# alibaba/TorchEasyRec

Hardware: NVIDIA H100
Metric: samples/sec (DLRM-Criteo synth, train step fwd+bwd+optimizer) (higher is better)
Workload: dtype f32

## Files before the change

### torcheasyrec_b200/csrc/build.py

```python

import os
import subprocess
import sys

HERE = os.path.dirname(os.path.abspath(__file__))
SOURCES = ["tzk_core.cu", "tzk_gather.cu", "tzk_bwd.cu", "tzk_dist.cu", "tzk_dense.cu", "tzk_tower.cu", "tzk_din.cu", "tzk_peer.cu", "tzk_interact_wide.cu",
           "tzk_interact_bf16.cu"]
HEADERS = ["tzk_common.cuh", "tzk_tower_bwd2.cuh", "tzk_interact_tc.cuh", "tzk_tower_tail.cuh", "tzk_interact_bf16.cuh",
"tzk_sm90_ptx.h", "tzk_tma.h", "tzk_wgrad3x.cuh", os.path.join("..", "..", "include", "tzk.h")]
LIB = os.path.join(HERE, "libtzk.so")
NVCC = os.environ.get("NVCC", "/usr/local/cuda/bin/nvcc")
FLAGS = [
    "-gencode", "arch=compute_90a,code=sm_90a",
    "-O3", "-lineinfo", "-std=c++17",
    "-Xcompiler", "-fPIC",
    "--expt-relaxed-constexpr",
]


def _mtime(p):
    return os.path.getmtime(p) if os.path.exists(p) else 0.0


def build(verbose: bool = False, force: bool = False) -> str:
    hdr_time = max(_mtime(os.path.join(HERE, h)) for h in HEADERS)
    objs = []
    procs = []
    for src in SOURCES:
        s = os.path.join(HERE, src)
        o = os.path.join(HERE, src.replace(".cu", ".o"))
        objs.append(o)
        if force or _mtime(o) < max(_mtime(s), hdr_time):
            cmd = [NVCC, *FLAGS, "-c", s, "-o", o]
            if verbose:
                cmd.insert(1, "-Xptxas")
                cmd.insert(2, "-v")
                print(" ".join(cmd), flush=True)
            procs.append((src, subprocess.Popen(cmd, stdout=subprocess.PIPE, stderr=subprocess.STDOUT, text=True)))
    failed = False
    for src, p in procs:
        out, _ = p.communicate()
        if p.returncode != 0:
            failed = True
            sys.stderr.write(f"nvcc failed for {src}:\n{out}\n")
        elif verbose and out:
            print(out)
    if failed:
        raise RuntimeError("libtzk build failed")
    if force or procs or _mtime(LIB) < max(_mtime(o) for o in objs):
        cmd = [NVCC, "-shared", "-Wno-deprecated-gpu-targets", "-o", LIB + ".tmp", *objs]
        subprocess.run(cmd, check=True)
        os.replace(LIB + ".tmp", LIB)
    build_gemm(force)
    build_gemm3x(force)
    return LIB


def build_gemm3x(force: bool = False) -> str:
    src = os.path.join(HERE, "tzk_gemm3x.cu")
    lib = os.path.join(HERE, "libtzk_gemm3x.so")
    deps = [src] + [os.path.join(HERE, h) for h in ("tzk_sm90_ptx.h", "tzk_tma.h", "tzk_wgrad3x.cuh")]
    if force or _mtime(lib) < max(_mtime(d) for d in deps):
        subprocess.run([NVCC, *FLAGS, "-shared", src, "-o", lib + ".tmp"], check=True)
        os.replace(lib + ".tmp", lib)
    return lib


def build_gemm(force: bool = False) -> str:
    src = os.path.join(HERE, "tzk_gemm.cpp")
    lib = os.path.join(HERE, "libtzk_gemm.so")
    if force or _mtime(lib) < _mtime(src):
        subprocess.run(["g++", "-O2", "-std=c++17", "-fPIC", "-shared", "-I/usr/local/cuda/include", src, "-o", lib,
                        "-ldl"], check=True)
    return lib


if __name__ == "__main__":
    print(build(verbose="-v" in sys.argv, force="-f" in sys.argv))
```

### torcheasyrec_b200/csrc/tzk_interact_wide.cu

```cuda
#include <stdint.h>
#include <stdio.h>
#include <stdlib.h>

#ifdef TZK_CPU_SHIM
#include "cuda_cpu_shim.h"
#include "sm90_cpu_emu.h"
typedef void* tzk_stream_t;
#define TZK_REQUIRE(cond, ...) do { if (!(cond)) return 1; } while (0)
#define TZK_CHECK_LAUNCH(name) do {} while (0)
#else
#include <cuda.h>
#include "tzk_common.cuh"
#define TZK_DYN_SMEM(type, name) extern __shared__ __align__(1024) type name[]
#define TZK_UNPAREN(...) __VA_ARGS__
#define TZK_LAUNCH(kernel, grid, block, smem, stream, ...) TZK_UNPAREN kernel<<<grid, block, smem, stream>>>(__VA_ARGS__)
#endif

namespace {
#ifndef TZK_CPU_SHIM
#include "tzk_sm90_ptx.h"
#endif
#include "tzk_tma.h"
namespace tzk_itc {
__device__ __forceinline__ uint32_t cvt_tf32(float x) { return tf32_bits(x); }
__device__ __forceinline__ void mma_tf32(float (&c)[4], const uint32_t (&a)[4], const uint32_t (&b)[2]) { ::mma_tf32(c, a, b); }
}
#include "tzk_interact_tc.cuh"

__device__ __forceinline__ float4 load_l2(const float* p) {
#ifdef TZK_CPU_SHIM
  return *reinterpret_cast<const float4*>(p);
#else
  return __ldcg(reinterpret_cast<const float4*>(p));
#endif
}

constexpr int FB_M = 64;
constexpr int FB_THREADS = 512;
constexpr int FB_WARPS = FB_THREADS / 32;
constexpr int FB_CHUNKS = (tzk_itc::kRow + 31) / 32;
constexpr int FB_PAIR_CHUNKS = tzk_itc::kInter / 32;
constexpr int FB_BOX = 32 * 128;
constexpr int FB_STAGE = 4 * FB_BOX;
constexpr int FB_STAGES = 3;
constexpr int FB_LDP = 360;
constexpr int FB_P_OFF = FB_STAGES * FB_STAGE;
constexpr int FB_S_OFF = FB_P_OFF + FB_M * FB_LDP * 4;
constexpr int FB_IJ_OFF = FB_S_OFF + FB_WARPS * 32 * tzk_itc::kSS * 4;
constexpr int FB_BAR_OFF = FB_IJ_OFF + tzk_itc::kInter * 2;
constexpr int FB_SMEM = FB_BAR_OFF + FB_STAGES * 8;

struct FbParams {
  const float* dz; int64_t ld_dz;
  const float* dense; int64_t ld_dense;
  const float* sparse; int64_t ld_sparse;
  float* d_dense; int64_t ld_ddense;
  float* d_sparse; int64_t ld_dsparse;
  int64_t M;
};

__global__ void __launch_bounds__(FB_THREADS, 1)
interact_wide_bwd_kernel(const __grid_constant__ CUtensorMap map_whi, const __grid_constant__ CUtensorMap map_wlo,
                         FbParams p) {
  TZK_DYN_SMEM(uint8_t, smem);
  float* P = reinterpret_cast<float*>(smem + FB_P_OFF);
  uint64_t* full = reinterpret_cast<uint64_t*>(smem + FB_BAR_OFF);
  const int warp = threadIdx.x >> 5, lane = threadIdx.x & 31, g = lane >> 2, t = lane & 3;
  const int64_t m0 = (int64_t)blockIdx.x * FB_M;

  if (threadIdx.x == 0) {
    for (int s = 0; s < FB_STAGES; ++s) mbar_init(full + s, 1);
    fence_mbarrier_init();
  }
  float* S = reinterpret_cast<float*>(smem + FB_S_OFF) + warp * (32 * tzk_itc::kSS);
  unsigned short* pair_ij = reinterpret_cast<unsigned short*>(smem + FB_IJ_OFF);
  tzk_itc::init_pair_ij(pair_ij);
  for (int i = lane; i < 32 * tzk_itc::kSS; i += 32) S[i] = 0.f;
  __syncthreads();
  auto col_chunk = [](int c) { return (c + FB_PAIR_CHUNKS) % FB_CHUNKS; };
  auto load = [&](int c) {
    uint8_t* sb = smem + (c % FB_STAGES) * FB_STAGE;
    uint64_t* bar = full + c % FB_STAGES;
    const int n0 = col_chunk(c) * 32;
    mbar_expect_tx(bar, FB_STAGE);
    tma_load_2d(sb, &map_whi, bar, 0, n0);
    tma_load_2d(sb + FB_BOX, &map_whi, bar, 32, n0);
    tma_load_2d(sb + 2 * FB_BOX, &map_wlo, bar, 0, n0);
    tma_load_2d(sb + 3 * FB_BOX, &map_wlo, bar, 32, n0);
  };
  if (threadIdx.x == 0)
    for (int c = 0; c < FB_STAGES; ++c) load(c);

  const int wm = warp & 3, wn = warp >> 2;
  const int r = wm * 16 + g;
  uint32_t ah[8][4], al[8][4];
#pragma unroll
  for (int kk = 0; kk < 8; ++kk) {
    const int k0 = kk * 8 + t, k1 = k0 + 4;
    const int64_t ra = m0 + r, rb = ra + 8;
    const float a[4] = {ra < p.M ? __ldg(p.dz + ra * p.ld_dz + k0) : 0.f, rb < p.M ? __ldg(p.dz + rb * p.ld_dz + k0) : 0.f,
                        ra < p.M ? __ldg(p.dz + ra * p.ld_dz + k1) : 0.f, rb < p.M ? __ldg(p.dz + rb * p.ld_dz + k1) : 0.f};
#pragma unroll
    for (int i = 0; i < 4; ++i) {
      ah[kk][i] = tf32_bits(a[i]);
      al[kk][i] = tf32_bits(a[i] - __uint_as_float(ah[kk][i]));
    }
  }
  const int n = wn * 8 + g;
  for (int c = 0; c < FB_CHUNKS; ++c) {
    const int s = c % FB_STAGES;
    mbar_wait(full + s, (uint32_t)(c / FB_STAGES) & 1u);
    const uint32_t* whi = reinterpret_cast<const uint32_t*>(smem + s * FB_STAGE);
    const uint32_t* wlo = whi + 2 * FB_BOX / 4;
    float acc[4] = {0.f, 0.f, 0.f, 0.f};
#pragma unroll
    for (int kk = 0; kk < 8; ++kk) {
      const uint32_t* bh_box = whi + (kk >> 2) * (FB_BOX / 4);
      const uint32_t* bl_box = wlo + (kk >> 2) * (FB_BOX / 4);
      const int k0 = (kk & 3) * 8 + t, k1 = k0 + 4;
      const uint32_t bh[2] = {bh_box[swz(n, k0)], bh_box[swz(n, k1)]};
      const uint32_t bl[2] = {bl_box[swz(n, k0)], bl_box[swz(n, k1)]};
      float part[4] = {0.f, 0.f, 0.f, 0.f};
      mma_tf32(part, al[kk], bh);
      mma_tf32(part, ah[kk], bl);
      mma_tf32(part, ah[kk], bh);
#pragma unroll
      for (int q = 0; q < 4; ++q) acc[q] += part[q];
    }
    const int col = col_chunk(c) * 32 + wn * 8 + 2 * t;
    if (col < tzk_itc::kInter) {
      *reinterpret_cast<float2*>(P + r * FB_LDP + col) = make_float2(acc[0], acc[1]);
      *reinterpret_cast<float2*>(P + (r + 8) * FB_LDP + col) = make_float2(acc[2], acc[3]);
    } else if (col < tzk_itc::kRow) {
      const int e = col - tzk_itc::kInter;
#pragma unroll
      for (int h = 0; h < 2; ++h) {
        const int64_t row = m0 + r + 8 * h;
        if (row >= p.M) continue;
        float* dst = e < tzk_itc::kD ? p.d_dense + row * p.ld_ddense + e : p.d_sparse + row * p.ld_dsparse + (e - tzk_itc::kD);
        *reinterpret_cast<float2*>(dst) = make_float2(acc[2 * h], acc[2 * h + 1]);
      }
    }
    __syncthreads();
    if (threadIdx.x == 0 && c + FB_STAGES < FB_CHUNKS) load(c + FB_STAGES);
  }

  for (int i = warp; i < FB_M; i += FB_WARPS) {
    const int64_t b = m0 + i;
    if (b >= p.M) break;
    float* dd = p.d_dense + b * p.ld_ddense;
    float* ds = p.d_sparse + b * p.ld_dsparse;
    float4 pass[4];
#pragma unroll
    for (int q = 0; q < 4; ++q) {
      const int row = g + 8 * q;
      pass[q] = row == 0 ? load_l2(dd + 4 * t)
              : row < tzk_itc::kN ? load_l2(ds + (row - 1) * tzk_itc::kD + 4 * t)
              : make_float4(0.f, 0.f, 0.f, 0.f);
    }
    tzk_itc::bwd_sample(P + i * FB_LDP, p.dense + b * p.ld_dense, p.sparse + b * p.ld_sparse, pass, pair_ij, S, dd, ds,
                        lane);
  }
}

constexpr int FF_M = 128;
constexpr int FF_THREADS = 256;
constexpr int FF_WARPS = FF_THREADS / 32;
constexpr int FF_X_BYTES = FF_M * 128;
constexpr int FF_W_BYTES = 64 * 128;
constexpr int FF_STAGE = FF_X_BYTES + 2 * FF_W_BYTES;
constexpr int FF_STAGES = 3;
constexpr int FF_E_OFF = FF_STAGES * FF_STAGE;
constexpr int FF_BAR_OFF = FF_E_OFF + FF_X_BYTES;
constexpr int FF_SMEM = FF_BAR_OFF + FF_STAGES * 8;
static_assert(FF_WARPS * tzk_itc::kInter * 4 <= FF_X_BYTES, "staging rows overflow their region");
constexpr int FF_SPARSE0 = tzk_itc::kInter + tzk_itc::kD;

struct FfParams {
  const float* dense; int64_t ld_dense;
  const float* sparse; int64_t ld_sparse;
  float* pairs; int64_t ld_pairs;
  const float* bias;
  float* y; int64_t ld_y;
  int64_t M;
};

__device__ __forceinline__ void fence_proxy_async() {
#ifndef TZK_CPU_SHIM
  asm volatile("fence.proxy.async;" ::: "memory");
#endif
}

__global__ void __launch_bounds__(FF_THREADS, 2)
interact_wide_fwd_kernel(const __grid_constant__ CUtensorMap map_pairs, const __grid_constant__ CUtensorMap map_dense,
                         const __grid_constant__ CUtensorMap map_sparse, const __grid_constant__ CUtensorMap map_whi, const __grid_constant__ CUtensorMap map_wlo,
                         FfParams p) {
  TZK_DYN_SMEM(uint8_t, smem);
  uint64_t* full = reinterpret_cast<uint64_t*>(smem + FF_BAR_OFF);
  const int warp = threadIdx.x >> 5, lane = threadIdx.x & 31, g = lane >> 2, t = lane & 3;
  const int64_t m0 = (int64_t)blockIdx.x * FF_M;
  const int64_t m_end = p.M - m0 < FF_M ? p.M : m0 + FF_M;

  if (threadIdx.x == 0) {
    for (int s = 0; s < FF_STAGES; ++s) mbar_init(full + s, 1);
    fence_mbarrier_init();
  }
  {
    float* O = reinterpret_cast<float*>(smem + FF_E_OFF) + warp * tzk_itc::kInter;
    if (lane == 0) O[tzk_itc::kP] = 0.f;
    int rowbase[4];
    tzk_itc::pair_rowbase(g, rowbase);
    int64_t b = m0 + warp;
    float4 x[4];
    if (b < m_end) {
#pragma unroll
      for (int j = 0; j < 4; ++j) x[j] = tzk_itc::load_x4(p.dense + b * p.ld_dense, p.sparse + b * p.ld_sparse, g + 8 * j, 4 * t);
    }
    for (; b < m_end; b += FF_WARPS) {
      float4 xn[4];
      const int64_t bn = b + FF_WARPS;
      if (bn < m_end) {
#pragma unroll
        for (int j = 0; j < 4; ++j)
          xn[j] = tzk_itc::load_x4(p.dense + bn * p.ld_dense, p.sparse + bn * p.ld_sparse, g + 8 * j, 4 * t);
      }
      tzk_itc::fwd_sample(x, rowbase, O, p.pairs + b * p.ld_pairs, lane);
      if (bn < m_end) {
#pragma unroll
        for (int j = 0; j < 4; ++j) x[j] = xn[j];
      }
    }
  }
  fence_proxy_async();
  __syncthreads();

  auto load = [&](int c) {
    uint8_t* sb = smem + (c % FF_STAGES) * FF_STAGE;
    uint64_t* bar = full + c % FF_STAGES;
    mbar_expect_tx(bar, c == FB_PAIR_CHUNKS ? FF_STAGE + FF_X_BYTES : FF_STAGE);
    if (c < FB_PAIR_CHUNKS) {
      tma_load_2d(sb, &map_pairs, bar, 32 * c, (int)m0);
    } else if (c == FB_PAIR_CHUNKS) {
      tma_load_2d(sb, &map_dense, bar, 0, (int)m0);
      tma_load_2d(smem + FF_E_OFF, &map_sparse, bar, 0, (int)m0);
    } else {
      tma_load_2d(sb, &map_sparse, bar, 32 * c - FF_SPARSE0, (int)m0);
    }
    tma_load_2d(sb + FF_X_BYTES, &map_whi, bar, 32 * c, 0);
    tma_load_2d(sb + FF_X_BYTES + FF_W_BYTES, &map_wlo, bar, 32 * c, 0);
  };
  if (threadIdx.x == 0)
    for (int c = 0; c < FF_STAGES; ++c) load(c);

  const int r = warp * 16 + g;
  float acc[8][4], part[8][4];
#pragma unroll
  for (int nt = 0; nt < 8; ++nt)
#pragma unroll
    for (int q = 0; q < 4; ++q) acc[nt][q] = 0.f;
  for (int c = 0; c < FB_CHUNKS; ++c) {
    const int s = c % FF_STAGES;
    mbar_wait(full + s, (uint32_t)(c / FF_STAGES) & 1u);
    const float* xs = reinterpret_cast<const float*>(smem + s * FF_STAGE);
    const uint32_t* whi = reinterpret_cast<const uint32_t*>(smem + s * FF_STAGE + FF_X_BYTES);
    const uint32_t* wlo = whi + FF_W_BYTES / 4;
#pragma unroll
    for (int ks = 0; ks < 4; ++ks) {
#pragma unroll
      for (int nt = 0; nt < 8; ++nt)
#pragma unroll
        for (int q = 0; q < 4; ++q) part[nt][q] = 0.f;
      const int k0 = ks * 8 + t, k1 = k0 + 4;
      const bool sp = ks >= 2 && c == FB_PAIR_CHUNKS;
      const float* as = sp ? reinterpret_cast<const float*>(smem + FF_E_OFF) : xs;
      const int x16 = sp ? 16 : 0;
      const float a[4] = {as[swz(r, k0) ^ x16], as[swz(r + 8, k0) ^ x16], as[swz(r, k1) ^ x16], as[swz(r + 8, k1) ^ x16]};
      uint32_t ah[4], al[4];
#pragma unroll
      for (int i = 0; i < 4; ++i) {
        ah[i] = tf32_bits(a[i]);
        al[i] = tf32_bits(a[i] - __uint_as_float(ah[i]));
      }
#pragma unroll
      for (int nt = 0; nt < 8; ++nt) {
        const int n = nt * 8 + g;
        const uint32_t bh[2] = {whi[swz(n, k0)], whi[swz(n, k1)]};
        const uint32_t bl[2] = {wlo[swz(n, k0)], wlo[swz(n, k1)]};
        mma_tf32(part[nt], al, bh);
        mma_tf32(part[nt], ah, bl);
        mma_tf32(part[nt], ah, bh);
      }
#pragma unroll
      for (int nt = 0; nt < 8; ++nt)
#pragma unroll
        for (int q = 0; q < 4; ++q) acc[nt][q] += part[nt][q];
    }
    __syncthreads();
    if (threadIdx.x == 0 && c + FF_STAGES < FB_CHUNKS) load(c + FF_STAGES);
  }
#pragma unroll
  for (int nt = 0; nt < 8; ++nt) {
    const int col = nt * 8 + 2 * t;
    const float b0 = p.bias ? __ldg(p.bias + col) : 0.f, b1 = p.bias ? __ldg(p.bias + col + 1) : 0.f;
#pragma unroll
    for (int h = 0; h < 2; ++h) {
      const int64_t row = m0 + r + 8 * h;
      if (row >= p.M) continue;
      float2 o = make_float2(acc[nt][2 * h] + b0, acc[nt][2 * h + 1] + b1);
      o.x = fmaxf(o.x, 0.f);
      o.y = fmaxf(o.y, 0.f);
      *reinterpret_cast<float2*>(p.y + row * p.ld_y + col) = o;
    }
  }
}

__global__ void split_w_kernel(const float* __restrict__ w, int64_t ld_w, int K, float* __restrict__ hi,
                               float* __restrict__ lo) {
  const int i = blockIdx.x * blockDim.x + threadIdx.x;
  if (i < K * 64) {
    const float v = w[(int64_t)(i / K) * ld_w + i % K];
    const float h = tf32_rna(v);
    hi[i] = h;
    lo[i] = tf32_rna(v - h);
  }
}

#include "tzk_wgrad3x.cuh"

__global__ void split_wt_kernel(const float* __restrict__ w, int64_t ld_w, int K, float* __restrict__ hi,
                                float* __restrict__ lo) {
  const int i = blockIdx.x * blockDim.x + threadIdx.x;
  if (i < K * 64) {
    const int k = i >> 6, o = i & 63;
    const float v = w[(int64_t)o * ld_w + k];
    const float h = tf32_rna(v);
    hi[i] = h;
    lo[i] = tf32_rna(v - h);
  }
}

}

extern "C" int tzk_interact_wide_bwd(const float* dz, int64_t ld_dz, const float* w, int64_t ld_w, const float* dense,
                                     int64_t ld_dense, const float* sparse, int64_t ld_sparse, int64_t M, float* d_dense,
                                     int64_t ld_ddense, float* d_sparse, int64_t ld_dsparse, float* wt_hi, float* wt_lo,
                                     tzk_stream_t stream) {
  TZK_REQUIRE(M > 0, "interact_wide_bwd: M must be positive");
  TZK_REQUIRE(ld_w >= tzk_itc::kRow, "interact_wide_bwd: w needs %d columns", tzk_itc::kRow);
  const int64_t lds[] = {ld_dz, ld_w, ld_dense, ld_sparse, ld_ddense, ld_dsparse};
  for (int64_t ld : lds) TZK_REQUIRE(ld % 4 == 0, "interact_wide_bwd: row strides must be multiples of 4 floats");
  const void* ptrs[] = {dz, w, dense, sparse, d_dense, d_sparse, wt_hi, wt_lo};
  for (const void* q : ptrs)
    TZK_REQUIRE(q && reinterpret_cast<uintptr_t>(q) % 16 == 0, "interact_wide_bwd: NULL or not 16-B aligned pointer");
  cudaStream_t st = reinterpret_cast<cudaStream_t>(stream);
  TZK_LAUNCH((split_wt_kernel), (tzk_itc::kRow * 64 + 255) / 256, 256, 0, st, w, ld_w, tzk_itc::kRow, wt_hi, wt_lo);
  CUtensorMap mh, ml;
  TZK_REQUIRE(!make_map(&mh, wt_hi, tzk_itc::kRow, 64, 64, 32) && !make_map(&ml, wt_lo, tzk_itc::kRow, 64, 64, 32),
              "interact_wide_bwd: tensor-map encoding failed");
  FbParams p;
  p.dz = dz; p.ld_dz = ld_dz; p.dense = dense; p.ld_dense = ld_dense; p.sparse = sparse; p.ld_sparse = ld_sparse;
  p.d_dense = d_dense; p.ld_ddense = ld_ddense; p.d_sparse = d_sparse; p.ld_dsparse = ld_dsparse; p.M = M;
#ifndef TZK_CPU_SHIM
  static bool configured = false;
  if (!configured) {
    cudaFuncSetAttribute(interact_wide_bwd_kernel, cudaFuncAttributeMaxDynamicSharedMemorySize, FB_SMEM);
    configured = true;
  }
#endif
  TZK_LAUNCH((interact_wide_bwd_kernel), (unsigned)((M + FB_M - 1) / FB_M), FB_THREADS, FB_SMEM, st, mh, ml, p);
  TZK_CHECK_LAUNCH("interact_wide_bwd_kernel");
  return 0;
}

extern "C" int tzk_interact_wide_fwd(const float* dense, int64_t ld_dense, const float* sparse, int64_t ld_sparse,
                                     const float* w, int64_t ld_w, const float* bias, int64_t M, float* y, int64_t ld_y,
                                     float* pairs, int64_t ld_pairs, float* w_hi, float* w_lo, tzk_stream_t stream) {
  TZK_REQUIRE(M > 0, "interact_wide_fwd: M must be positive");
  TZK_REQUIRE(ld_w >= tzk_itc::kRow && ld_y >= 64 && ld_pairs >= tzk_itc::kInter && ld_dense >= tzk_itc::kD &&
              ld_sparse >= tzk_itc::kRow - FF_SPARSE0, "interact_wide_fwd: row stride shorter than the row");
  const int64_t lds[] = {ld_dense, ld_sparse, ld_w, ld_y, ld_pairs};
  for (int64_t ld : lds) TZK_REQUIRE(ld % 4 == 0, "interact_wide_fwd: row strides must be multiples of 4 floats");
  const void* ptrs[] = {dense, sparse, w, y, pairs, w_hi, w_lo};
  for (const void* q : ptrs)
    TZK_REQUIRE(q && reinterpret_cast<uintptr_t>(q) % 16 == 0, "interact_wide_fwd: NULL or not 16-B aligned pointer");
  cudaStream_t st = reinterpret_cast<cudaStream_t>(stream);
  TZK_LAUNCH((split_w_kernel), (tzk_itc::kRow * 64 + 255) / 256, 256, 0, st, w, ld_w, tzk_itc::kRow, w_hi, w_lo);
  CUtensorMap mp, md, ms, mh, ml;
  TZK_REQUIRE(!make_map(&mp, pairs, M, tzk_itc::kInter, ld_pairs, FF_M) &&
              !make_map(&md, dense, M, tzk_itc::kD, ld_dense, FF_M) &&
              !make_map(&ms, sparse, M, tzk_itc::kRow - FF_SPARSE0, ld_sparse, FF_M) &&
              !make_map(&mh, w_hi, 64, tzk_itc::kRow, tzk_itc::kRow, 64) &&
              !make_map(&ml, w_lo, 64, tzk_itc::kRow, tzk_itc::kRow, 64), "interact_wide_fwd: tensor-map encoding failed");
  FfParams p;
  p.dense = dense; p.ld_dense = ld_dense; p.sparse = sparse; p.ld_sparse = ld_sparse; p.pairs = pairs;
  p.ld_pairs = ld_pairs; p.bias = bias; p.y = y; p.ld_y = ld_y; p.M = M;
#ifndef TZK_CPU_SHIM
  static bool configured = false;
  if (!configured) {
    cudaFuncSetAttribute(interact_wide_fwd_kernel, cudaFuncAttributeMaxDynamicSharedMemorySize, FF_SMEM);
    configured = true;
  }
#endif
  TZK_LAUNCH((interact_wide_fwd_kernel), (unsigned)((M + FF_M - 1) / FF_M), FF_THREADS, FF_SMEM, st, mp, md, ms, mh, ml, p);
  TZK_CHECK_LAUNCH("interact_wide_fwd_kernel");
  return 0;
}

extern "C" int tzk_interact_wide_wgrad(const float* dz, int64_t ld_dz, const float* pairs, int64_t ld_pairs,
                                       const float* dense, int64_t ld_dense, const float* sparse, int64_t ld_sparse,
                                       int64_t M, int32_t slabs, float* partial, float* dw, int64_t ld_dw,
                                       tzk_stream_t stream) {
  TZK_REQUIRE(M > 0 && slabs > 0, "interact_wide_wgrad: M and slabs must be positive");
  TZK_REQUIRE(ld_dw >= tzk_itc::kRow, "interact_wide_wgrad: dw needs %d columns", tzk_itc::kRow);
  const int64_t lds[] = {ld_dz, ld_pairs, ld_dense, ld_sparse};
  for (int64_t ld : lds) TZK_REQUIRE(ld % 4 == 0, "interact_wide_wgrad: row strides must be multiples of 4 floats");
  const void* ptrs[] = {dz, pairs, dense, sparse, partial, dw};
  for (const void* q : ptrs)
    TZK_REQUIRE(q && reinterpret_cast<uintptr_t>(q) % 16 == 0, "interact_wide_wgrad: NULL or not 16-B aligned pointer");
  CUtensorMap mx[WG_SRC], mz;
  TZK_REQUIRE(!make_map(&mx[0], pairs, M, tzk_itc::kInter, ld_pairs, WG_ROWS) &&
              !make_map(&mx[1], sparse, M, tzk_itc::kRow - FF_SPARSE0, ld_sparse, WG_ROWS) &&
              !make_map(&mx[2], dense, M, tzk_itc::kD, ld_dense, WG_ROWS) &&
              !make_map(&mz, dz, M, 64, ld_dz, WG_ROWS), "interact_wide_wgrad: tensor-map encoding failed");
  const WgSources src = {{0, FB_PAIR_CHUNKS, FB_CHUNKS - 1, FB_CHUNKS}, {0, 0, 0}, {0, FF_SPARSE0, tzk_itc::kInter},
                         {tzk_itc::kInter, tzk_itc::kRow - FF_SPARSE0, tzk_itc::kD}};
  TZK_REQUIRE(wgrad3x_launch(mx, mz, src, M, slabs, partial, dw, ld_dw, reinterpret_cast<cudaStream_t>(stream)) == 0,
              "interact_wide_wgrad: launch failed");
  return 0;
}
```

### torcheasyrec_b200/csrc/tzk_wgrad3x.cuh

```cuda
#pragma once

constexpr int WG_THREADS = 256;
constexpr int WG_ROWS = 32;
constexpr int WG_BOX = WG_ROWS * 128;
constexpr int WG_A = 4 * WG_BOX, WG_B = 2 * WG_BOX;
constexpr int WG_STAGE = WG_A + WG_B;
constexpr int WG_STAGES = 4;
constexpr int WG_SRC = 3;

struct WgSources {
  int first[WG_SRC + 1];
  int col0[WG_SRC];
  int dst[WG_SRC];
  int width[WG_SRC];
};

struct WgParams {
  float* partial;
  int64_t M;
  int64_t slab_rows;
  int k_tiles;
  WgSources src;
};

__device__ __forceinline__ int wg_source(const WgSources& s, int box) {
  return box >= s.first[2] ? 2 : box >= s.first[1] ? 1 : 0;
}
__device__ __forceinline__ int wg_pick(const int* v, int s) { return s == 0 ? v[0] : s == 1 ? v[1] : v[2]; }

__global__ void __launch_bounds__(WG_THREADS, 2)
wgrad3x_kernel(const __grid_constant__ CUtensorMap map_x0, const __grid_constant__ CUtensorMap map_x1,
               const __grid_constant__ CUtensorMap map_x2, const __grid_constant__ CUtensorMap map_dz, WgParams p) {
  TZK_DYN_SMEM(uint8_t, smem);
  uint64_t* full = reinterpret_cast<uint64_t*>(smem + WG_STAGES * WG_STAGE);
  int* boxes = reinterpret_cast<int*>(full + WG_STAGES);

  const int warp = threadIdx.x >> 5, lane = threadIdx.x & 31, g = lane >> 2, t = lane & 3;
  const int jt = blockIdx.x % p.k_tiles;
  const int64_t slab = blockIdx.x / p.k_tiles;
  const int64_t row0 = slab * p.slab_rows;
  const int64_t rows = (p.M - row0 < p.slab_rows) ? p.M - row0 : p.slab_rows;
  const int num_c = (int)((rows + WG_ROWS - 1) / WG_ROWS);

  if (threadIdx.x == 0) {
    for (int s = 0; s < WG_STAGES; ++s) mbar_init(full + s, 1);
    fence_mbarrier_init();
    for (int b = 0; b < 4; ++b) {
      const int box = jt * 4 + b, s = wg_source(p.src, box);
      boxes[b] = s;
      boxes[4 + b] = wg_pick(p.src.col0, s) + 32 * (box - wg_pick(p.src.first, s));
    }
  }
  __syncthreads();
  auto load = [&](int c) {
    uint8_t* sb = smem + (c % WG_STAGES) * WG_STAGE;
    uint64_t* bar = full + c % WG_STAGES;
    const int r = (int)(row0 + (int64_t)c * WG_ROWS);
    mbar_expect_tx(bar, WG_A + WG_B);
#pragma unroll 1
    for (int b = 0; b < 4; ++b) {
      const int s = *reinterpret_cast<volatile int*>(boxes + b), col = *reinterpret_cast<volatile int*>(boxes + 4 + b);
      tma_load_2d(sb + b * WG_BOX, s == 0 ? &map_x0 : s == 1 ? &map_x1 : &map_x2, bar, col, r);
    }
#pragma unroll
    for (int b = 0; b < 2; ++b) tma_load_2d(sb + WG_A + b * WG_BOX, &map_dz, bar, b * 32, r);
  };
  if (threadIdx.x == 0)
    for (int c = 0; c < WG_STAGES && c < num_c; ++c) load(c);

  const int n0 = (warp & 3) * 16 + g;
  const int kc0 = (warp >> 2) * 64 + g;
  float acc[8][4], part[8][4];
#pragma unroll
  for (int nt = 0; nt < 8; ++nt)
#pragma unroll
    for (int q = 0; q < 4; ++q) acc[nt][q] = 0.f;
  for (int c = 0; c < num_c; ++c) {
    const int s = c % WG_STAGES;
    mbar_wait(full + s, (uint32_t)(c / WG_STAGES) & 1u);
    const float* xs = reinterpret_cast<const float*>(smem + s * WG_STAGE);
    const float* zs = reinterpret_cast<const float*>(smem + s * WG_STAGE + WG_A);
    auto at = [](const float* base, int m, int col) { return base[(col >> 5) * (WG_BOX / 4) + swz(m, col & 31)]; };
#pragma unroll
    for (int ks = 0; ks < WG_ROWS / 8; ++ks) {
#pragma unroll
      for (int nt = 0; nt < 8; ++nt)
#pragma unroll
        for (int q = 0; q < 4; ++q) part[nt][q] = 0.f;
      const int m = ks * 8 + t;
      const float a[4] = {at(zs, m, n0), at(zs, m, n0 + 8), at(zs, m + 4, n0), at(zs, m + 4, n0 + 8)};
      uint32_t ah[4], al[4];
#pragma unroll
      for (int i = 0; i < 4; ++i) {
        ah[i] = tf32_bits(a[i]);
        al[i] = tf32_bits(a[i] - __uint_as_float(ah[i]));
      }
#pragma unroll
      for (int nt = 0; nt < 8; ++nt) {
        const float b[2] = {at(xs, m, kc0 + 8 * nt), at(xs, m + 4, kc0 + 8 * nt)};
        uint32_t bh[2], bl[2];
#pragma unroll
        for (int i = 0; i < 2; ++i) {
          bh[i] = tf32_bits(b[i]);
          bl[i] = tf32_bits(b[i] - __uint_as_float(bh[i]));
        }
        mma_tf32(part[nt], al, bh);
        mma_tf32(part[nt], ah, bl);
        mma_tf32(part[nt], ah, bh);
      }
#pragma unroll
      for (int nt = 0; nt < 8; ++nt)
#pragma unroll
        for (int q = 0; q < 4; ++q) acc[nt][q] += part[nt][q];
    }
    __syncthreads();
    if (threadIdx.x == 0 && c + WG_STAGES < num_c) load(c + WG_STAGES);
  }
  float* out = p.partial + ((int64_t)slab * p.k_tiles + jt) * 128 * 64;
#pragma unroll
  for (int nt = 0; nt < 8; ++nt) {
    const int kcol = (warp >> 2) * 64 + nt * 8 + 2 * t;
#pragma unroll
    for (int q = 0; q < 4; ++q) out[(int64_t)(kcol + (q & 1)) * 64 + n0 + 8 * (q >> 1)] = acc[nt][q];
  }
}

__global__ void wgrad_reduce_kernel(const float* __restrict__ partial, int slabs, int k_pad, WgSources src,
                                    float* __restrict__ dw, int64_t ld_dw) {
  const int i = blockIdx.x * blockDim.x + threadIdx.x;
  if (i >= k_pad * 64) return;
  const int k = i >> 6, n = i & 63;
  const int s = wg_source(src, k >> 5);
  const int c = k - 32 * wg_pick(src.first, s);
  if (c >= wg_pick(src.width, s)) return;
  float acc = 0.f;
  for (int sl = 0; sl < slabs; ++sl) acc += partial[((int64_t)sl * k_pad + k) * 64 + n];
  dw[(int64_t)n * ld_dw + wg_pick(src.dst, s) + c] = acc;
}

inline int wgrad3x_launch(const CUtensorMap (&mx)[WG_SRC], const CUtensorMap& mz, const WgSources& src, int64_t M,
                          int32_t slabs, float* partial, float* dw, int64_t ld_dw, cudaStream_t st) {
  WgParams p;
  p.partial = partial;
  p.M = M;
  p.k_tiles = (src.first[WG_SRC] + 3) / 4;
  p.slab_rows = ((M + slabs - 1) / slabs + WG_ROWS - 1) / WG_ROWS * WG_ROWS;
  p.src = src;
  const int used = (int)((M + p.slab_rows - 1) / p.slab_rows);
  const size_t smem = (size_t)WG_STAGES * WG_STAGE + WG_STAGES * 8 + 8 * 4;
#ifndef TZK_CPU_SHIM
  static bool configured = false;
  if (!configured) {
    cudaFuncSetAttribute(wgrad3x_kernel, cudaFuncAttributeMaxDynamicSharedMemorySize, (int)smem);
    configured = true;
  }
#endif
  TZK_LAUNCH((wgrad3x_kernel), used * p.k_tiles, WG_THREADS, smem, st, mx[0], mx[1], mx[2], mz, p);
  TZK_LAUNCH((wgrad_reduce_kernel), (p.k_tiles * 128 * 64 + 255) / 256, 256, 0, st, partial, used, p.k_tiles * 128, src,
             dw, ld_dw);
  return cudaGetLastError() == cudaSuccess ? 0 : 3;
}
```

Before: 45.83 million.

## Use wgmma 3xTF32 for interact-wide forward and weight-gradient GEMMs

Replaces the warp-level mma.sync 3xTF32 loops in the interact-wide forward kernel with Hopper wgmma m64n64k8 instructions that read the B operand (weight hi/lo) directly from swizzled shared memory through descriptors. Adds a dedicated weight-gradient kernel that splits dz into tf32 hi/lo transposed tiles in shared memory each chunk, then issues wgmma against them, and templatizes the wgrad launcher to accept this kernel and its extra smem. The aim is to cut shared-memory fragment loads and per-warp MMA issue overhead. In exchange it adds an extra smem staging pass and syncs per chunk, raises smem use (which can lower occupancy), and waits on each wgmma group immediately, so there is little async overlap.

```diff
diff --git a/torcheasyrec_b200/csrc/build.py b/torcheasyrec_b200/csrc/build.py
--- a/torcheasyrec_b200/csrc/build.py
+++ b/torcheasyrec_b200/csrc/build.py
@@ -7,7 +7,7 @@
 SOURCES = ["tzk_core.cu", "tzk_gather.cu", "tzk_bwd.cu", "tzk_dist.cu", "tzk_dense.cu", "tzk_tower.cu", "tzk_din.cu", "tzk_peer.cu", "tzk_interact_wide.cu",
            "tzk_interact_bf16.cu"]
 HEADERS = ["tzk_common.cuh", "tzk_tower_bwd2.cuh", "tzk_interact_tc.cuh", "tzk_tower_tail.cuh", "tzk_interact_bf16.cuh",
-"tzk_sm90_ptx.h", "tzk_tma.h", "tzk_wgrad3x.cuh", os.path.join("..", "..", "include", "tzk.h")]
+"tzk_sm90_ptx.h", "tzk_tma.h", "tzk_wgrad3x.cuh", "tzk_wgmma.cuh", os.path.join("..", "..", "include", "tzk.h")]
 LIB = os.path.join(HERE, "libtzk.so")
 NVCC = os.environ.get("NVCC", "/usr/local/cuda/bin/nvcc")
 FLAGS = [
diff --git a/torcheasyrec_b200/csrc/tzk_interact_wide.cu b/torcheasyrec_b200/csrc/tzk_interact_wide.cu
--- a/torcheasyrec_b200/csrc/tzk_interact_wide.cu
+++ b/torcheasyrec_b200/csrc/tzk_interact_wide.cu
@@ -5,6 +5,7 @@
 #ifdef TZK_CPU_SHIM
 #include "cuda_cpu_shim.h"
 #include "sm90_cpu_emu.h"
+#include "sm90_wgmma_emu.h"
 typedef void* tzk_stream_t;
 #define TZK_REQUIRE(cond, ...) do { if (!(cond)) return 1; } while (0)
 #define TZK_CHECK_LAUNCH(name) do {} while (0)
@@ -21,6 +22,7 @@
 #include "tzk_sm90_ptx.h"
 #endif
 #include "tzk_tma.h"
+#include "tzk_wgmma.cuh"
 namespace tzk_itc {
 __device__ __forceinline__ uint32_t cvt_tf32(float x) { return tf32_bits(x); }
 __device__ __forceinline__ void mma_tf32(float (&c)[4], const uint32_t (&a)[4], const uint32_t (&b)[2]) { ::mma_tf32(c, a, b); }
@@ -253,23 +255,17 @@
     for (int c = 0; c < FF_STAGES; ++c) load(c);
 
   const int r = warp * 16 + g;
-  float acc[8][4], part[8][4];
-#pragma unroll
-  for (int nt = 0; nt < 8; ++nt)
-#pragma unroll
-    for (int q = 0; q < 4; ++q) acc[nt][q] = 0.f;
+  float acc[32], part[32];
+#pragma unroll
+  for (int i = 0; i < 32; ++i) acc[i] = 0.f;
   for (int c = 0; c < FB_CHUNKS; ++c) {
     const int s = c % FF_STAGES;
     mbar_wait(full + s, (uint32_t)(c / FF_STAGES) & 1u);
     const float* xs = reinterpret_cast<const float*>(smem + s * FF_STAGE);
-    const uint32_t* whi = reinterpret_cast<const uint32_t*>(smem + s * FF_STAGE + FF_X_BYTES);
-    const uint32_t* wlo = whi + FF_W_BYTES / 4;
+    const uint8_t* whi = smem + s * FF_STAGE + FF_X_BYTES;
+    const uint8_t* wlo = whi + FF_W_BYTES;
 #pragma unroll
     for (int ks = 0; ks < 4; ++ks) {
-#pragma unroll
-      for (int nt = 0; nt < 8; ++nt)
-#pragma unroll
-        for (int q = 0; q < 4; ++q) part[nt][q] = 0.f;
       const int k0 = ks * 8 + t, k1 = k0 + 4;
       const bool sp = ks >= 2 && c == FB_PAIR_CHUNKS;
       const float* as = sp ? reinterpret_cast<const float*>(smem + FF_E_OFF) : xs;
@@ -281,19 +277,15 @@
         ah[i] = tf32_bits(a[i]);
         al[i] = tf32_bits(a[i] - __uint_as_float(ah[i]));
       }
-#pragma unroll
-      for (int nt = 0; nt < 8; ++nt) {
-        const int n = nt * 8 + g;
-        const uint32_t bh[2] = {whi[swz(n, k0)], whi[swz(n, k1)]};
-        const uint32_t bl[2] = {wlo[swz(n, k0)], wlo[swz(n, k1)]};
-        mma_tf32(part[nt], al, bh);
-        mma_tf32(part[nt], ah, bl);
-        mma_tf32(part[nt], ah, bh);
-      }
-#pragma unroll
-      for (int nt = 0; nt < 8; ++nt)
-#pragma unroll
-        for (int q = 0; q < 4; ++q) acc[nt][q] += part[nt][q];
+      wgmma_fence();
+      wgmma_3xtf32<64>(part, ah, al, wgmma_desc(whi, ks), wgmma_desc(wlo, ks));
+      wgmma_commit();
+      wgmma_wait<0>();
+#pragma unroll
+      for (int i = 0; i < 32; ++i) {
+        wgmma_reg_fence(part[i]);
+        acc[i] += part[i];
+      }
     }
     __syncthreads();
     if (threadIdx.x == 0 && c + FF_STAGES < FB_CHUNKS) load(c + FF_STAGES);
@@ -306,7 +298,7 @@
     for (int h = 0; h < 2; ++h) {
       const int64_t row = m0 + r + 8 * h;
       if (row >= p.M) continue;
-      float2 o = make_float2(acc[nt][2 * h] + b0, acc[nt][2 * h + 1] + b1);
+      float2 o = make_float2(acc[4 * nt + 2 * h] + b0, acc[4 * nt + 2 * h + 1] + b1);
       o.x = fmaxf(o.x, 0.f);
       o.y = fmaxf(o.y, 0.f);
       *reinterpret_cast<float2*>(p.y + row * p.ld_y + col) = o;
@@ -326,6 +318,112 @@
 }
 
 #include "tzk_wgrad3x.cuh"
+
+constexpr int WW_ZT = 64 * 128;
+
+__global__ void __launch_bounds__(WG_THREADS, 2)
+interact_wide_wgrad_kernel(const __grid_constant__ CUtensorMap map_x0, const __grid_constant__ CUtensorMap map_x1,
+                           const __grid_constant__ CUtensorMap map_x2, const __grid_constant__ CUtensorMap map_dz,
+                           WgParams p) {
+  TZK_DYN_SMEM(uint8_t, smem);
+  uint8_t* zt = smem + WG_STAGES * WG_STAGE;
+  uint64_t* full = reinterpret_cast<uint64_t*>(zt + 2 * WW_ZT);
+  int* boxes = reinterpret_cast<int*>(full + WG_STAGES);
+
+  const int warp = threadIdx.x >> 5, lane = threadIdx.x & 31, g = lane >> 2, t = lane & 3;
+  const int jt = blockIdx.x % p.k_tiles;
+  const int64_t slab = blockIdx.x / p.k_tiles;
+  const int64_t row0 = slab * p.slab_rows;
+  const int64_t rows = (p.M - row0 < p.slab_rows) ? p.M - row0 : p.slab_rows;
+  const int num_c = (int)((rows + WG_ROWS - 1) / WG_ROWS);
+
+  if (threadIdx.x == 0) {
+    for (int s = 0; s < WG_STAGES; ++s) mbar_init(full + s, 1);
+    fence_mbarrier_init();
+    for (int b = 0; b < 4; ++b) {
+      const int box = jt * 4 + b, s = wg_source(p.src, box);
+      boxes[b] = s;
+      boxes[4 + b] = wg_pick(p.src.col0, s) + 32 * (box - wg_pick(p.src.first, s));
+    }
+  }
+  __syncthreads();
+  auto load = [&](int c) {
+    uint8_t* sb = smem + (c % WG_STAGES) * WG_STAGE;
+    uint64_t* bar = full + c % WG_STAGES;
+    const int r = (int)(row0 + (int64_t)c * WG_ROWS);
+    mbar_expect_tx(bar, WG_A + WG_B);
+#pragma unroll 1
+    for (int b = 0; b < 4; ++b) {
+      const int s = *reinterpret_cast<volatile int*>(boxes + b), col = *reinterpret_cast<volatile int*>(boxes + 4 + b);
+      tma_load_2d(sb + b * WG_BOX, s == 0 ? &map_x0 : s == 1 ? &map_x1 : &map_x2, bar, col, r);
+    }
+#pragma unroll
+    for (int b = 0; b < 2; ++b) tma_load_2d(sb + WG_A + b * WG_BOX, &map_dz, bar, b * 32, r);
+  };
+  if (threadIdx.x == 0)
+    for (int c = 0; c < WG_STAGES && c < num_c; ++c) load(c);
+
+  const int xc = (warp >> 2) * 64 + (warp & 3) * 16 + g;
+  const int tn = threadIdx.x & 63, tq = threadIdx.x >> 6;
+  uint32_t* zhi = reinterpret_cast<uint32_t*>(zt);
+  uint32_t* zlo = zhi + WW_ZT / 4;
+  float acc[32], part[32];
+#pragma unroll
+  for (int i = 0; i < 32; ++i) acc[i] = 0.f;
+  for (int c = 0; c < num_c; ++c) {
+    const int s = c % WG_STAGES;
+    mbar_wait(full + s, (uint32_t)(c / WG_STAGES) & 1u);
+    const float* xs = reinterpret_cast<const float*>(smem + s * WG_STAGE);
+    const float* zs = reinterpret_cast<const float*>(smem + s * WG_STAGE + WG_A);
+    auto at = [](const float* base, int m, int col) { return base[(col >> 5) * (WG_BOX / 4) + swz(m, col & 31)]; };
+#pragma unroll
+    for (int h = 0; h < 2; ++h) {
+      const int m = 4 * tq + 16 * h;
+      float hi[4], lo[4];
+#pragma unroll
+      for (int j = 0; j < 4; ++j) {
+        const float v = at(zs, m + j, tn);
+        hi[j] = tf32_rna(v);
+        lo[j] = tf32_rna(v - hi[j]);
+      }
+      *reinterpret_cast<float4*>(zhi + swz(tn, m)) = make_float4(hi[0], hi[1], hi[2], hi[3]);
+      *reinterpret_cast<float4*>(zlo + swz(tn, m)) = make_float4(lo[0], lo[1], lo[2], lo[3]);
+    }
+    fence_proxy_async();
+    __syncthreads();
+#pragma unroll
+    for (int ks = 0; ks < WG_ROWS / 8; ++ks) {
+      const int m = ks * 8 + t;
+      const float a[4] = {at(xs, m, xc), at(xs, m, xc + 8), at(xs, m + 4, xc), at(xs, m + 4, xc + 8)};
+      uint32_t ah[4], al[4];
+#pragma unroll
+      for (int i = 0; i < 4; ++i) {
+        ah[i] = tf32_bits(a[i]);
+        al[i] = tf32_bits(a[i] - __uint_as_float(ah[i]));
+      }
+      wgmma_fence();
+      wgmma_tf32<64>(part, ah, wgmma_desc(zlo, ks), false);
+      wgmma_tf32<64>(part, al, wgmma_desc(zhi, ks), true);
+      wgmma_tf32<64>(part, ah, wgmma_desc(zhi, ks), true);
+      wgmma_commit();
+      wgmma_wait<0>();
+#pragma unroll
+      for (int i = 0; i < 32; ++i) {
+        wgmma_reg_fence(part[i]);
+        acc[i] += part[i];
+      }
+    }
+    __syncthreads();
+    if (threadIdx.x == 0 && c + WG_STAGES < num_c) load(c + WG_STAGES);
+  }
+  float* out = p.partial + ((int64_t)slab * p.k_tiles + jt) * 128 * 64;
+#pragma unroll
+  for (int i = 0; i < 8; ++i)
+#pragma unroll
+    for (int h = 0; h < 2; ++h)
+      *reinterpret_cast<float2*>(out + (int64_t)(xc + 8 * h) * 64 + 8 * i + 2 * t) =
+          make_float2(acc[4 * i + 2 * h], acc[4 * i + 2 * h + 1]);
+}
 
 __global__ void split_wt_kernel(const float* __restrict__ w, int64_t ld_w, int K, float* __restrict__ hi,
                                 float* __restrict__ lo) {
@@ -424,7 +522,8 @@
               !make_map(&mz, dz, M, 64, ld_dz, WG_ROWS), "interact_wide_wgrad: tensor-map encoding failed");
   const WgSources src = {{0, FB_PAIR_CHUNKS, FB_CHUNKS - 1, FB_CHUNKS}, {0, 0, 0}, {0, FF_SPARSE0, tzk_itc::kInter},
                          {tzk_itc::kInter, tzk_itc::kRow - FF_SPARSE0, tzk_itc::kD}};
-  TZK_REQUIRE(wgrad3x_launch(mx, mz, src, M, slabs, partial, dw, ld_dw, reinterpret_cast<cudaStream_t>(stream)) == 0,
+  TZK_REQUIRE(wgrad3x_launch<interact_wide_wgrad_kernel>(mx, mz, src, M, slabs, partial, dw, ld_dw,
+                                                         reinterpret_cast<cudaStream_t>(stream), 2 * WW_ZT) == 0,
               "interact_wide_wgrad: launch failed");
   return 0;
 }
diff --git a/torcheasyrec_b200/csrc/tzk_wgmma.cuh b/torcheasyrec_b200/csrc/tzk_wgmma.cuh
--- /dev/null
+++ b/torcheasyrec_b200/csrc/tzk_wgmma.cuh
@@ -0,0 +1,39 @@
+#pragma once
+
+__device__ __forceinline__ uint64_t wgmma_desc(const void* box, int ks) {
+  const uint32_t a = smem_u32(box) + 32u * (uint32_t)ks;
+  return (uint64_t)((a >> 4) & 0x3fffu) | (1ull << 16) | ((uint64_t)(1024 >> 4) << 32) | (1ull << 62);
+}
+
+#ifndef TZK_CPU_SHIM
+__device__ __forceinline__ void wgmma_fence() { asm volatile("wgmma.fence.sync.aligned;" ::: "memory"); }
+__device__ __forceinline__ void wgmma_commit() { asm volatile("wgmma.commit_group.sync.aligned;" ::: "memory"); }
+template <int N>
+__device__ __forceinline__ void wgmma_wait() { asm volatile("wgmma.wait_group.sync.aligned %0;" ::"n"(N) : "memory"); }
+__device__ __forceinline__ void wgmma_reg_fence(float& r) { asm volatile("" : "+f"(r)::"memory"); }
+
+template <int N>
+__device__ __forceinline__ void wgmma_tf32(float (&d)[N / 2], const uint32_t (&a)[4], uint64_t desc, bool scale_d);
+
+template <>
+__device__ __forceinline__ void wgmma_tf32<64>(float (&d)[32], const uint32_t (&a)[4], uint64_t desc, bool scale_d) {
+  asm volatile(
+      "{\n\t.reg .pred p;\n\tsetp.ne.b32 p, %37, 0;\n\t"
+      "wgmma.mma_async.sync.aligned.m64n64k8.f32.tf32.tf32 "
+      "{%0,%1,%2,%3,%4,%5,%6,%7,%8,%9,%10,%11,%12,%13,%14,%15,"
+      "%16,%17,%18,%19,%20,%21,%22,%23,%24,%25,%26,%27,%28,%29,%30,%31}, {%32,%33,%34,%35}, %36, p, 1, 1;\n\t}"
+      : "+f"(d[0]), "+f"(d[1]), "+f"(d[2]), "+f"(d[3]), "+f"(d[4]), "+f"(d[5]), "+f"(d[6]), "+f"(d[7]),
+        "+f"(d[8]), "+f"(d[9]), "+f"(d[10]), "+f"(d[11]), "+f"(d[12]), "+f"(d[13]), "+f"(d[14]), "+f"(d[15]),
+        "+f"(d[16]), "+f"(d[17]), "+f"(d[18]), "+f"(d[19]), "+f"(d[20]), "+f"(d[21]), "+f"(d[22]), "+f"(d[23]),
+        "+f"(d[24]), "+f"(d[25]), "+f"(d[26]), "+f"(d[27]), "+f"(d[28]), "+f"(d[29]), "+f"(d[30]), "+f"(d[31])
+      : "r"(a[0]), "r"(a[1]), "r"(a[2]), "r"(a[3]), "l"(desc), "r"((int)scale_d));
+}
+#endif
+
+template <int N>
+__device__ __forceinline__ void wgmma_3xtf32(float (&part)[N / 2], const uint32_t (&ah)[4], const uint32_t (&al)[4],
+                                             uint64_t hi_b, uint64_t lo_b) {
+  wgmma_tf32<N>(part, al, hi_b, false);
+  wgmma_tf32<N>(part, ah, lo_b, true);
+  wgmma_tf32<N>(part, ah, hi_b, true);
+}
diff --git a/torcheasyrec_b200/csrc/tzk_wgrad3x.cuh b/torcheasyrec_b200/csrc/tzk_wgrad3x.cuh
--- a/torcheasyrec_b200/csrc/tzk_wgrad3x.cuh
+++ b/torcheasyrec_b200/csrc/tzk_wgrad3x.cuh
@@ -138,8 +138,10 @@
   dw[(int64_t)n * ld_dw + wg_pick(src.dst, s) + c] = acc;
 }
 
+template <auto Kernel = wgrad3x_kernel>
 inline int wgrad3x_launch(const CUtensorMap (&mx)[WG_SRC], const CUtensorMap& mz, const WgSources& src, int64_t M,
-                          int32_t slabs, float* partial, float* dw, int64_t ld_dw, cudaStream_t st) {
+                          int32_t slabs, float* partial, float* dw, int64_t ld_dw, cudaStream_t st,
+                          size_t extra_smem = 0) {
   WgParams p;
   p.partial = partial;
   p.M = M;
@@ -147,15 +149,15 @@
   p.slab_rows = ((M + slabs - 1) / slabs + WG_ROWS - 1) / WG_ROWS * WG_ROWS;
   p.src = src;
   const int used = (int)((M + p.slab_rows - 1) / p.slab_rows);
-  const size_t smem = (size_t)WG_STAGES * WG_STAGE + WG_STAGES * 8 + 8 * 4;
+  const size_t smem = (size_t)WG_STAGES * WG_STAGE + extra_smem + WG_STAGES * 8 + 8 * 4;
 #ifndef TZK_CPU_SHIM
   static bool configured = false;
   if (!configured) {
-    cudaFuncSetAttribute(wgrad3x_kernel, cudaFuncAttributeMaxDynamicSharedMemorySize, (int)smem);
+    cudaFuncSetAttribute(Kernel, cudaFuncAttributeMaxDynamicSharedMemorySize, (int)smem);
     configured = true;
   }
 #endif
-  TZK_LAUNCH((wgrad3x_kernel), used * p.k_tiles, WG_THREADS, smem, st, mx[0], mx[1], mx[2], mz, p);
+  TZK_LAUNCH((Kernel), used * p.k_tiles, WG_THREADS, smem, st, mx[0], mx[1], mx[2], mz, p);
   TZK_LAUNCH((wgrad_reduce_kernel), (p.k_tiles * 128 * 64 + 255) / 256, 256, 0, st, partial, used, p.k_tiles * 128, src,
              dw, ld_dw);
   return cudaGetLastError() == cudaSuccess ? 0 : 3;
```

Measured after the change: 50.87 million (median of 6 runs). 1.11x the previous value.
